# PeihaoChen/RSPNet

Hardware: AMD Instinct MI355X
Metric: clips/sec pretext step (c3d 16x112x112, B=32/GPU) (higher is better)
Workload: dtype f32

## Files before the change

rspnet_amd/csrc/common.h:

```cpp
#pragma once
#include <hip/hip_runtime.h>
#include <stdint.h>
#include <stdio.h>
#include <stdlib.h>
#include <string.h>
#include <tuple>

#include "rspnet_hip.h"

typedef float floatx16 __attribute__((ext_vector_type(16)));
typedef float floatx4 __attribute__((ext_vector_type(4)));

#define RSP_WAVE 64

void rsp_set_error(const char* msg);
void rsp_note_reset(void);
void rsp_note_kernel(const char* fmt, ...);

static inline int rsp_check_launch(const char* what) {
  hipError_t e = hipGetLastError();
  if (e != hipSuccess) {
    char buf[256];
    snprintf(buf, sizeof buf, "%.*s: %s", (int)strcspn(what, "<"), what, hipGetErrorString(e));
    rsp_set_error(buf);
    return RSP_ELAUNCH;
  }
  return RSP_OK;
}

#define RSP_CONV_OPTIONS(X)                                                             \
  X(OPT_NARROW_MAX_TILES, "narrow_max_tiles", "RSP_NARROW_MAX_TILES", 0, 512)           \
  X(OPT_NARROW32_MAX_UNITS, "narrow32_max_units", "RSP_NARROW32_MAX_UNITS", 0, 256)     \
  X(OPT_TALL_MIN_TILES, "tall_min_tiles", "RSP_TALL_MIN_TILES", 0, 0)                   \
  X(OPT_TWO_LEVEL_MIN_CHUNKS, "two_level_min_chunks", "RSP_TWO_LEVEL_MIN_CHUNKS", 0, 0) \
  X(OPT_DIRECT_MAX_TILES, "direct_max_tiles", "RSP_DIRECT_MAX_TILES", 0, 0)             \
  X(OPT_NO_PERSIST, "no_persist", "RSP_NO_PERSIST", 1, 0)                               \
  X(OPT_NO_HALF_BLOCK, "no_half_block", "RSP_NO_HALF_BLOCK", 1, 0)                      \
  X(OPT_NO_PAD_SKIP, "no_pad_skip", "RSP_NO_PAD_SKIP", 1, 0)                            \
  X(OPT_NO_DMAJOR, "no_dmajor", "RSP_NO_DMAJOR", 1, 0)                                  \
  X(OPT_NO_TM_SKIP, "no_tm_skip", "RSP_NO_TM_SKIP", 1, 0)                               \
  X(OPT_NO_MULTI_SPLIT, "no_multi_split", "RSP_NO_MULTI_SPLIT", 1, 0)
#define RSP_OPTION_ID(id, name, env, flag, dflt) id,
enum RspConvOption { RSP_CONV_OPTIONS(RSP_OPTION_ID) RSP_OPT_COUNT };
#undef RSP_OPTION_ID
int rsp_conv_option(RspConvOption id);

template <auto KERNEL, class... Args, class... Note>
int rsp_launch_lds(dim3 grid, size_t lds, size_t lds_max, hipStream_t s, const std::tuple<Args...>& args, const char* fmt, Note... note) {
  static bool attr_set = false;
  if (!attr_set) {
    (void)hipFuncSetAttribute(reinterpret_cast<const void*>(KERNEL), hipFuncAttributeMaxDynamicSharedMemorySize, (int)lds_max);
    attr_set = true;
  }
  rsp_note_kernel(fmt, note...);
  std::apply([&](const auto&... a) { hipLaunchKernelGGL(KERNEL, grid, dim3(256), lds, s, a...); }, args);
  return rsp_check_launch(fmt);
}

#define RSP_REQUIRE(cond, msg)     \
  do {                             \
    if (!(cond)) {                 \
      rsp_set_error(msg);          \
      return RSP_EINVAL;           \
    }                              \
  } while (0)

static inline size_t rsp_align_up(size_t v, size_t a) { return (v + a - 1) / a * a; }
static inline int rsp_cdiv(int64_t a, int64_t b) { return (int)((a + b - 1) / b); }
static inline bool rsp_aligned16(const void* p) { return (((uintptr_t)p) & 15) == 0; }

__device__ __forceinline__ int rsp_xcd_remap(int bid, int nwg) {
  const int q = nwg >> 3, r = nwg & 7;
  const int xcd = bid & 7;
  const int base = xcd < r ? xcd * (q + 1) : r * (q + 1) + (xcd - r) * q;
  return base + (bid >> 3);
}

__device__ __forceinline__ float rsp_wave_sum(float v) {
#pragma unroll
  for (int o = 32; o > 0; o >>= 1) v += __shfl_xor(v, o);
  return v;
}
__device__ __forceinline__ int rsp_wave_sum_i(int v) {
#pragma unroll
  for (int o = 32; o > 0; o >>= 1) v += __shfl_xor(v, o);
  return v;
}
__device__ __forceinline__ double rsp_wave_sum_d(double v) {
#pragma unroll
  for (int o = 32; o > 0; o >>= 1) v += __shfl_xor(v, o);
  return v;
}
__device__ __forceinline__ float rsp_wave_max(float v) {
#pragma unroll
  for (int o = 32; o > 0; o >>= 1) v = fmaxf(v, __shfl_xor(v, o));
  return v;
}

__device__ __forceinline__ float rsp_max_nan(float best, float v) { return __builtin_elementwise_maximum(best, v); }
__device__ __forceinline__ float rsp_relu(float z) { return __builtin_elementwise_maximum(z, 0.f); }
__device__ __forceinline__ bool rsp_relu_blocks(float z) { return z <= 0.f; }
__device__ __forceinline__ bool rsp_max_takes(float v, float best) { return v > best || v != v; }
__device__ __forceinline__ bool rsp_max_displaced(bool earlier, float v, float mine) {
  const bool vn = v != v, mn = mine != mine;
  return earlier ? (!mn && (vn || v >= mine)) : (vn || (!mn && v > mine));
}

struct FastDiv {
  unsigned mul;
  unsigned shr;
  int d;
};

static inline FastDiv fastdiv_make(int d) {
  FastDiv f = {0u, 0u, d};
  if (d <= 1) return f;
  int s = 0;
  while ((1ll << s) < d) ++s;
  const unsigned long long pw = 1ull << (31 + s);
  f.mul = (unsigned)((pw + (unsigned long long)d - 1) / (unsigned long long)d);
  f.shr = (unsigned)(s - 1);
  return f;
}

__device__ __forceinline__ int fastdiv(int n, const FastDiv f) {
  return f.mul ? (int)(__umulhi((unsigned)n, f.mul) >> f.shr) : n;
}
```

rspnet_amd/csrc/conv_stem.hip:

```cpp
#include "conv_stem.h"

#include <mutex>
#include <unordered_map>

namespace {

struct StemParams {
  const float* __restrict__ x;
  const float* __restrict__ w;
  const float* __restrict__ bias;
  float* __restrict__ y;
  float* __restrict__ stat;
  int N, Di, Hi, Wi, Do, Ho, Wo;
  int kT, kH, kW, sT, sH, sW, pT, pH, pW;
  int Cout, out_ld;
  int tw_shift;
  int HT, WT, WTh, WTL;
  int npix, npix_r;
  int FR;
  int ntaps, nchunks;
  int tiles_h, tiles_w, tiles;
  unsigned x_bytes, w_bytes;
  int wide;
  float* __restrict__ ymax;
  float* __restrict__ ymin;
  int pool_ld;
};

struct StemBias {
  floatx4 w[2];
  float n[2];
};

__device__ __forceinline__ StemBias stem_bias(const float* __restrict__ bias, int Cout, bool wide, int lane) {
  StemBias b;
#pragma unroll
  for (int j = 0; j < 2; ++j) {
    b.w[j] = floatx4{0.f, 0.f, 0.f, 0.f};
    b.n[j] = 0.f;
    const int cw = 32 * j + 4 * (lane & 7), cn = 32 * j + (lane & 31);
    if (bias && wide && cw < Cout) b.w[j] = *reinterpret_cast<const floatx4*>(bias + cw);
    if (bias && !wide && cn < Cout) b.n[j] = bias[cn];
  }
  asm volatile("" : "+v"(b.w[0]), "+v"(b.w[1]), "+v"(b.n[0]), "+v"(b.n[1]));
  return b;
}

__device__ __forceinline__ void stem_store_wide(const StemParams& p, const floatx16 (&acc)[2], float* stage ,
                                                const long long* rowaddr , int wave, int lane, const StemBias& b) {
  const int l32 = lane & 31, h = lane >> 5;
  const int q = lane & 7, rbase = lane >> 3;
#pragma unroll
  for (int j = 0; j < 2; ++j) {
    const int col = 32 * j + 4 * q;
#pragma unroll
    for (int r = 0; r < 2; ++r) {
#pragma unroll
      for (int e = 0; e < 8; ++e) stage[((e >> 2) * 8 + h * 4 + (e & 3)) * 32 + l32] = acc[j][8 * r + e];
#pragma unroll
      for (int i = 0; i < 2; ++i) {
        const int rl = rbase + 8 * i;
        const floatx4 v = *reinterpret_cast<const floatx4*>(stage + rl * 32 + 4 * q);
        const long long addr = rowaddr[wave * 32 + 16 * r + rl];
        if (addr >= 0 && col < p.Cout) *reinterpret_cast<floatx4*>(p.y + addr + col) = v + b.w[j];
      }
    }
  }
}

__device__ __forceinline__ void stem_store_pooled(const StemParams& p, const floatx16 (&acc)[2], float* stage ,
                                                  int n, int to, int h0, int w0, int wave, int lane, const StemBias& b) {
  const int l32 = lane & 31, h = lane >> 5;
  const int q = lane & 15, kr = lane >> 4;
  long long addr[2];
#pragma unroll
  for (int i = 0; i < 2; ++i) {
    const int ho = h0 + 2 * wave, wo = w0 + 2 * (kr + 4 * i);
    addr[i] = (ho < p.Ho && wo < p.Wo && 4 * q < p.Cout)
                  ? ((((long long)n * p.Do + to) * (p.Ho >> 1) + (ho >> 1)) * (p.Wo >> 1) + (wo >> 1)) * p.pool_ld + 4 * q
                  : -1;
  }
#pragma unroll
  for (int o = 0; o < 2; ++o) {
#pragma unroll
    for (int j = 0; j < 2; ++j)
#pragma unroll
      for (int e0 = 0; e0 < 8; e0 += 2) {
        const float v0 = acc[j][e0] + b.n[j], v1 = acc[j][e0 + 1] + b.n[j], v2 = acc[j][e0 + 8] + b.n[j], v3 = acc[j][e0 + 9] + b.n[j];
        const float r = o == 0 ? __builtin_elementwise_maximum(__builtin_elementwise_maximum(v0, v1), __builtin_elementwise_maximum(v2, v3))
                               : __builtin_elementwise_minimum(__builtin_elementwise_minimum(v0, v1), __builtin_elementwise_minimum(v2, v3));
        stage[((e0 >> 2) * 4 + h * 2 + ((e0 & 3) >> 1)) * 64 + 32 * j + l32] = r;
      }
    float* dst = o == 0 ? p.ymax : p.ymin;
#pragma unroll
    for (int i = 0; i < 2; ++i) {
      const floatx4 v = *reinterpret_cast<const floatx4*>(stage + (kr + 4 * i) * 64 + 4 * q);
      if (addr[i] >= 0) *reinterpret_cast<floatx4*>(dst + addr[i]) = v;
    }
  }
}

template <int G, int NS>
__global__ __launch_bounds__(256, 2) void stem_kernel(const StemParams p) {
  constexpr int TCH = 2 * G;
  constexpr int BU = TCH * 64;
  constexpr int BI = (BU + 255) / 256;
  typedef __attribute__((address_space(3))) void* lptr_t;
  extern __shared__ __attribute__((aligned(16))) unsigned char smem_raw[];
  float* halo = reinterpret_cast<float*>(smem_raw);
  float* Bs = halo + p.FR * p.npix_r * 4;
  int* taptab = reinterpret_cast<int*>(Bs + 2 * BU * 4);
  long long* rowaddr = reinterpret_cast<long long*>(taptab + p.nchunks * TCH);

  const int t = threadIdx.x;
  const int lane = t & 63;
  const int wave = __builtin_amdgcn_readfirstlane(t >> 6);
  const int l32 = lane & 31, h = lane >> 5;

  const int tile = rsp_xcd_remap(blockIdx.x, gridDim.x);
  const int wb = tile % p.tiles_w;
  int q0 = tile / p.tiles_w;
  const int hb = q0 % p.tiles_h;
  q0 /= p.tiles_h;
  const int to = q0 % p.Do;
  const int n = q0 / p.Do;
  const int TW = 1 << p.tw_shift, TH = 128 >> p.tw_shift;
  const int h0 = hb * TH, w0 = wb * TW;
  const StemBias bias = stem_bias(p.bias, p.Cout, p.wide != 0, lane);

  const int khw = p.kH * p.kW;
  for (int i = t; i < p.nchunks * TCH; i += 256) {
    int off = 0;
    if (i < p.ntaps) {
      const int kw = i % p.kW, r = i / p.kW;
      const int kh = r % p.kH, kt = r / p.kH;
      const int col = p.sW == 2 ? (kw & 1) * p.WTh + (kw >> 1) : kw;
      off = (((kt % p.FR) * p.npix_r) + kh * p.WTL + col) * 16;
    }
    taptab[i] = off;
  }

  unsigned hrel[4];
#pragma unroll
  for (int i = 0; i < 4; ++i) {
    const int q = i * 256 + t;
    unsigned r = 0xffffffffu;
    if (q < p.npix) {
      const int hyy = q / p.WTL, cc = q - hyy * p.WTL;
      const int wxp = p.sW == 2 ? (cc < p.WTh ? 2 * cc : 2 * (cc - p.WTh) + 1) : cc;
      const int hi = h0 * p.sH - p.pH + hyy, wi = w0 * p.sW - p.pW + wxp;
      if (wxp < p.WT && (unsigned)hi < (unsigned)p.Hi && (unsigned)wi < (unsigned)p.Wi) r = (unsigned)((hi * p.Wi + wi) * 16);
    }
    hrel[i] = r;
  }

  __amdgpu_buffer_rsrc_t rsrc_x = __builtin_amdgcn_make_buffer_rsrc(const_cast<float*>(p.x), 0, (int)p.x_bytes, 0x00020000);
  __amdgpu_buffer_rsrc_t rsrc_w = __builtin_amdgcn_make_buffer_rsrc(const_cast<float*>(p.w), 0, (int)p.w_bytes, 0x00020000);

  auto load_frame = [&](int f) {
    const int ti = to * p.sT - p.pT + f;
    const bool okf = (unsigned)ti < (unsigned)p.Di;
    const unsigned fbase = (unsigned)(((long long)(n * p.Di + (okf ? ti : 0)) * p.Hi * p.Wi) * 16);
    const int slot = f % p.FR;
#pragma unroll
    for (int i = 0; i < 4; ++i) {
      if (i * 256 + wave * 64 < p.npix_r) {
        const unsigned off = (okf & (hrel[i] != 0xffffffffu)) ? fbase + hrel[i] : 0xffffffffu;
        float* dst = halo + (slot * p.npix_r + i * 256 + wave * 64) * 4;
        __builtin_amdgcn_raw_ptr_buffer_load_lds(rsrc_x, (lptr_t)dst, 16, off, 0, 0, 0);
      }
    }
  };
  auto load_weights = [&](int c, int buf) {
#pragma unroll
    for (int i = 0; i < BI; ++i) {
      if (i * 256 + wave * 64 < BU) {
        const unsigned off = ((unsigned)c * BU + i * 256 + t) * 16u;
        float* dst = Bs + (buf * BU + i * 256 + wave * 64) * 4;
        __builtin_amdgcn_raw_ptr_buffer_load_lds(rsrc_w, (lptr_t)dst, 16, off, 0, 0, 0);
      }
    }
  };
  auto frame_hi = [&](int c) { return min(p.kT - 1, (c * TCH + TCH - 1) / khw); };

  int loaded = frame_hi(0);
  for (int f = 0; f <= loaded; ++f) load_frame(f);
  load_weights(0, 0);
  __syncthreads();

  const int m = wave * 32 + l32;
  const int hy = m >> p.tw_shift, wx = m & (TW - 1);
  const char* arow = reinterpret_cast<const char*>(halo) + ((hy * p.sH) * p.WTL + wx) * 16;
  int toff[G];
#pragma unroll
  for (int g = 0; g < G; ++g) toff[g] = taptab[2 * g + h];

  floatx16 acc[2];
#pragma unroll
  for (int j = 0; j < 2; ++j)
#pragma unroll
    for (int e = 0; e < 16; ++e) acc[j][e] = 0.f;

  int buf = 0;
  for (int c = 0; c < p.nchunks; ++c) {
    const bool more = c + 1 < p.nchunks;
    floatx4 af[G], bf[G][2];
#pragma unroll
    for (int g = 0; g < G; ++g) af[g] = *reinterpret_cast<const floatx4*>(arow + toff[g]);
    const float* bb = Bs + buf * BU * 4 + (h * 64 + l32) * 4;
#pragma unroll
    for (int g = 0; g < G; ++g)
#pragma unroll
      for (int j = 0; j < 2; ++j) bf[g][j] = *reinterpret_cast<const floatx4*>(bb + (2 * g * 64 + 32 * j) * 4);
    int toffn[G];
#pragma unroll
    for (int g = 0; g < G; ++g) toffn[g] = more ? taptab[(c + 1) * TCH + 2 * g + h] : 0;
    if (more) {
      load_weights(c + 1, buf ^ 1);
      const int fh = frame_hi(c + 1);
      while (loaded < fh) load_frame(++loaded);
    }
#pragma unroll
    for (int g = 0; g < G; ++g)
#pragma unroll
      for (int s = 0; s < NS; ++s)
#pragma unroll
        for (int j = 0; j < 2; ++j) acc[j] = __builtin_amdgcn_mfma_f32_32x32x2f32(af[g][s], bf[g][j][s], acc[j], 0, 0, 0);
    __builtin_amdgcn_sched_barrier(0);
    __syncthreads();
    buf ^= 1;
#pragma unroll
    for (int g = 0; g < G; ++g) toff[g] = toffn[g];
  }

  if (t < 128) {
    const int ry = t >> p.tw_shift, rx = t & (TW - 1);
    const int ho = h0 + ry, wo = w0 + rx;
    rowaddr[t] = (ho < p.Ho && wo < p.Wo) ? ((((long long)n * p.Do + to) * p.Ho + ho) * p.Wo + wo) * p.out_ld : -1;
  }
  __syncthreads();
  float* red = Bs;
  if (p.wide) stem_store_wide(p, acc, Bs + 512 + wave * 512, rowaddr, wave, lane, bias);
#pragma unroll
  for (int j = 0; j < 2; ++j) {
    const int col = 32 * j + l32;
    const float bv = bias.n[j];
    float s = 0.f, ss = 0.f;
#pragma unroll
    for (int e = 0; e < 16; ++e) {
      const long long addr = rowaddr[wave * 32 + (e >> 2) * 8 + h * 4 + (e & 3)];
      const float v = addr >= 0 ? acc[j][e] : 0.f;
      if (!p.wide && addr >= 0 && col < p.Cout) p.y[addr + col] = v + bv;
      s += v;
      ss = fmaf(v, v, ss);
    }
    s += __shfl_xor(s, 32);
    ss += __shfl_xor(ss, 32);
    if (h == 0) {
      red[(wave * 64 + col) * 2 + 0] = s;
      red[(wave * 64 + col) * 2 + 1] = ss;
    }
  }
  if (p.stat) {
    __syncthreads();
    if (t < 64 && t < p.Cout) {
      float s = 0.f, ss = 0.f;
#pragma unroll
      for (int w = 0; w < 4; ++w) {
        s += red[(w * 64 + t) * 2 + 0];
        ss += red[(w * 64 + t) * 2 + 1];
      }
      float* o = p.stat + ((long long)tile * p.Cout + t) * 2;
      o[0] = s;
      o[1] = ss;
    }
  }
}

template <int G, bool WIDE, int NS, bool POOL = false>
__global__ __launch_bounds__(256, 2) void stem_resident_kernel(const StemParams p) {
  constexpr int TCH = 2 * G;
  constexpr int BU = TCH * 64;
  constexpr int BI = (BU + 255) / 256;
  typedef __attribute__((address_space(3))) void* lptr_t;
  extern __shared__ __attribute__((aligned(16))) unsigned char smem_raw[];
  const int hsz = p.FR * p.npix_r * 4;
  float* halo = reinterpret_cast<float*>(smem_raw);
  float* Bs = halo + 2 * hsz;
  int* taptab = reinterpret_cast<int*>(Bs + p.nchunks * BU * 4);
  long long* rowaddr = reinterpret_cast<long long*>(taptab + p.nchunks * TCH);
  float* red = reinterpret_cast<float*>(rowaddr + 128);

  const int t = threadIdx.x;
  const int lane = t & 63;
  const int wave = __builtin_amdgcn_readfirstlane(t >> 6);
  const int l32 = lane & 31, h = lane >> 5;
  const int TW = 1 << p.tw_shift, TH = 128 >> p.tw_shift;

  for (int i = t; i < p.nchunks * TCH; i += 256) {
    int off = 0;
    if (i < p.ntaps) {
      const int kw = i % p.kW, r = i / p.kW;
      const int kh = r % p.kH, kt = r / p.kH;
      const int col = p.sW == 2 ? (kw & 1) * p.WTh + (kw >> 1) : kw;
      off = ((kt * p.npix_r) + kh * p.WTL + col) * 16;
    }
    taptab[i] = off;
  }
  __amdgpu_buffer_rsrc_t rsrc_x = __builtin_amdgcn_make_buffer_rsrc(const_cast<float*>(p.x), 0, (int)p.x_bytes, 0x00020000);
  __amdgpu_buffer_rsrc_t rsrc_w = __builtin_amdgcn_make_buffer_rsrc(const_cast<float*>(p.w), 0, (int)p.w_bytes, 0x00020000);
  for (int c = 0; c < p.nchunks; ++c) {
#pragma unroll
    for (int i = 0; i < BI; ++i) {
      if (i * 256 + wave * 64 < BU) {
        const unsigned off = ((unsigned)c * BU + i * 256 + t) * 16u;
        float* dst = Bs + (c * BU + i * 256 + wave * 64) * 4;
        __builtin_amdgcn_raw_ptr_buffer_load_lds(rsrc_w, (lptr_t)dst, 16, off, 0, 0, 0);
      }
    }
  }
  int hyy[4], wxp[4];
#pragma unroll
  for (int i = 0; i < 4; ++i) {
    const int q = i * 256 + t;
    hyy[i] = -(1 << 20);
    wxp[i] = 0;
    if (q < p.npix) {
      const int r = q / p.WTL, cc = q - r * p.WTL;
      const int wx_ = p.sW == 2 ? (cc < p.WTh ? 2 * cc : 2 * (cc - p.WTh) + 1) : cc;
      if (wx_ < p.WT) {
        hyy[i] = r;
        wxp[i] = wx_;
      }
    }
  }
  auto issue_halo = [&](int tile, int buf) {
    const int wb = tile % p.tiles_w;
    int q0 = tile / p.tiles_w;
    const int hb = q0 % p.tiles_h;
    q0 /= p.tiles_h;
    const int to = q0 % p.Do, n = q0 / p.Do;
    const int hi0 = hb * TH * p.sH - p.pH, wi0 = wb * TW * p.sW - p.pW;
    unsigned hrel[4];
#pragma unroll
    for (int i = 0; i < 4; ++i) {
      const int hi = hi0 + hyy[i], wi = wi0 + wxp[i];
      hrel[i] = ((unsigned)hi < (unsigned)p.Hi && (unsigned)wi < (unsigned)p.Wi) ? (unsigned)((hi * p.Wi + wi) * 16) : 0xffffffffu;
    }
    for (int f = 0; f < p.kT; ++f) {
      const int ti = to * p.sT - p.pT + f;
      const bool okf = (unsigned)ti < (unsigned)p.Di;
      const unsigned fbase = (unsigned)(((long long)(n * p.Di + (okf ? ti : 0)) * p.Hi * p.Wi) * 16);
#pragma unroll
      for (int i = 0; i < 4; ++i) {
        if (i * 256 + wave * 64 < p.npix_r) {
          const unsigned off = (okf & (hrel[i] != 0xffffffffu)) ? fbase + hrel[i] : 0xffffffffu;
          float* dst = halo + buf * hsz + (f * p.npix_r + i * 256 + wave * 64) * 4;
          __builtin_amdgcn_raw_ptr_buffer_load_lds(rsrc_x, (lptr_t)dst, 16, off, 0, 0, 0);
        }
      }
    }
  };

  const int m = wave * 32 + l32;
  const int rowoff = (((m >> p.tw_shift) * p.sH) * p.WTL + (m & (TW - 1))) * 16;
  const StemBias bias = stem_bias(p.bias, p.Cout, WIDE, lane);

  int cur = 0;
  if ((int)blockIdx.x < p.tiles) issue_halo(blockIdx.x, 0);
  for (int tile = blockIdx.x; tile < p.tiles; tile += gridDim.x) {
    __syncthreads();
    const int next = tile + gridDim.x;
    const char* arow = reinterpret_cast<const char*>(halo + cur * hsz) + rowoff;
    floatx16 acc[2];
#pragma unroll
    for (int j = 0; j < 2; ++j)
#pragma unroll
      for (int e = 0; e < 16; ++e) acc[j][e] = 0.f;
    for (int c = 0; c < p.nchunks; ++c) {
      floatx4 af[G], bf[G][2];
#pragma unroll
      for (int g = 0; g < G; ++g) af[g] = *reinterpret_cast<const floatx4*>(arow + taptab[c * TCH + 2 * g + h]);
      const float* bb = Bs + c * BU * 4 + (h * 64 + l32) * 4;
#pragma unroll
      for (int g = 0; g < G; ++g)
#pragma unroll
        for (int j = 0; j < 2; ++j) bf[g][j] = *reinterpret_cast<const floatx4*>(bb + (2 * g * 64 + 32 * j) * 4);
      if (c == p.nchunks - 1 && next < p.tiles) issue_halo(next, cur ^ 1);
#pragma unroll
      for (int g = 0; g < G; ++g)
#pragma unroll
        for (int s = 0; s < NS; ++s)
#pragma unroll
          for (int j = 0; j < 2; ++j) acc[j] = __builtin_amdgcn_mfma_f32_32x32x2f32(af[g][s], bf[g][j][s], acc[j], 0, 0, 0);
    }
    const int wb = tile % p.tiles_w;
    int q0 = tile / p.tiles_w;
    const int hb = q0 % p.tiles_h;
    q0 /= p.tiles_h;
    const int to = q0 % p.Do, n = q0 / p.Do;
    if (t < 128) {
      const int ho = hb * TH + (t >> p.tw_shift), wo = wb * TW + (t & (TW - 1));
      rowaddr[t] = (ho < p.Ho && wo < p.Wo) ? ((((long long)n * p.Do + to) * p.Ho + ho) * p.Wo + wo) * p.out_ld : -1;
    }
    __syncthreads();
    if (WIDE) stem_store_wide(p, acc, halo + cur * hsz + wave * 512, rowaddr, wave, lane, bias);
    if (POOL) stem_store_pooled(p, acc, halo + cur * hsz + wave * 512, n, to, hb * TH, wb * TW, wave, lane, bias);
#pragma unroll
    for (int j = 0; j < 2; ++j) {
      const int col = 32 * j + l32;
      const float bv = bias.n[j];
      float s = 0.f, ss = 0.f;
#pragma unroll
      for (int e = 0; e < 16; ++e) {
        const long long addr = rowaddr[wave * 32 + (e >> 2) * 8 + h * 4 + (e & 3)];
        const float v = addr >= 0 ? acc[j][e] : 0.f;
        if (!WIDE && !POOL && addr >= 0 && col < p.Cout) p.y[addr + col] = v + bv;
        s += v;
        ss = fmaf(v, v, ss);
      }
      s += __shfl_xor(s, 32);
      ss += __shfl_xor(ss, 32);
      if (h == 0) {
        red[(wave * 64 + col) * 2 + 0] = s;
        red[(wave * 64 + col) * 2 + 1] = ss;
      }
    }
    if (p.stat) {
      __syncthreads();
      if (t < 64 && t < p.Cout) {
        float s = 0.f, ss = 0.f;
#pragma unroll
        for (int w = 0; w < 4; ++w) {
          s += red[(w * 64 + t) * 2 + 0];
          ss += red[(w * 64 + t) * 2 + 1];
        }
        float* o = p.stat + ((long long)tile * p.Cout + t) * 2;
        o[0] = s;
        o[1] = ss;
      }
    }
    cur ^= 1;
  }
}

__global__ void stem_pack_kernel(const float* __restrict__ w, float* __restrict__ out, int Cout, int kT, int kH, int kW,
                                 int ntaps, long long total) {
  for (long long i = blockIdx.x * (long long)blockDim.x + threadIdx.x; i < total; i += (long long)gridDim.x * blockDim.x) {
    const int ci = (int)(i & 3), n = (int)((i >> 2) & 63), tap = (int)(i >> 8);
    float v = 0.f;
    if (tap < ntaps && n < Cout) {
      const int kw = tap % kW, r = tap / kW;
      const int kh = r % kH, kt = r / kH;
      v = w[((((long long)n * 4 + ci) * kT + kt) * kH + kh) * kW + kw];
    }
    out[i] = v;
  }
}

struct StemPlan {
  bool ok;
  int G, TCH, nchunks, tw_shift, HT, WT, WTh, WTL, npix, npix_r, FR, tiles_h, tiles_w;
  bool resident;
  bool wide_ok;
  long long tiles;
  size_t lds;
};

StemPlan stem_plan(const rsp_conv3d_desc* d) {
  StemPlan s;
  memset(&s, 0, sizeof s);
  if (d->Cin != 4 || d->in_ld != 4 || d->Cout > 64 || d->out_ld < d->Cout) return s;
  if (d->sW < 1 || d->sW > 2 || d->sH < 1 || d->sH > 2) return s;
  const int ntaps = d->kT * d->kH * d->kW;
  if (ntaps > 343) return s;
  if ((unsigned long long)d->N * d->Di * d->Hi * d->Wi * 16ull >= 0xF0000000ull) return s;
  const long long waste16 = (long long)rsp_cdiv(d->Ho, 8) * 8 * rsp_cdiv(d->Wo, 16) * 16;
  const long long waste8 = (long long)rsp_cdiv(d->Ho, 16) * 16 * rsp_cdiv(d->Wo, 8) * 8;
  s.tw_shift = waste8 < waste16 ? 3 : 4;
  const long long covered = waste8 < waste16 ? waste8 : waste16;
  if (ntaps > 64 && covered * 100 > (long long)d->Ho * d->Wo * 104) return s;
  const int TW = 1 << s.tw_shift, TH = 128 >> s.tw_shift;
  s.HT = (TH - 1) * d->sH + d->kH;
  s.WT = (TW - 1) * d->sW + d->kW;
  s.WTh = (s.WT + 1) / 2;
  s.WTL = d->sW == 2 ? 2 * s.WTh : s.WT;
  s.npix = s.HT * s.WTL;
  if (s.npix > 1024) return s;
  s.npix_r = (s.npix + 63) / 64 * 64;
  s.FR = d->kT < 3 ? d->kT : 3;
  int best = 0, best_pad = 1 << 30;
  const int cand[3] = {8, 7, 5};
  for (int i = 0; i < 3; ++i) {
    const int tch = 2 * cand[i];
    if (d->kT > 3 && d->kH * d->kW < 2 * tch) continue;
    const int pad = rsp_cdiv(ntaps, tch) * tch;
    if (pad < best_pad) {
      best_pad = pad;
      best = cand[i];
    }
  }
  if (!best) return s;
  s.G = best;
  s.TCH = 2 * best;
  s.nchunks = rsp_cdiv(ntaps, s.TCH);
  s.tiles_h = rsp_cdiv(d->Ho, TH);
  s.tiles_w = rsp_cdiv(d->Wo, TW);
  s.tiles = (long long)d->N * d->Do * s.tiles_h * s.tiles_w;
  if (s.tiles >= (1ll << 31)) return s;
  const size_t lds_res = (size_t)2 * d->kT * s.npix_r * 16 + (size_t)s.nchunks * s.TCH * 1024 + (size_t)s.nchunks * s.TCH * 4 +
                         128 * 8 + 2048;
  s.resident = d->kT <= 3 && lds_res <= 78 * 1024;
  s.lds = s.resident ? lds_res
                     : (size_t)s.FR * s.npix_r * 16 + (size_t)2 * s.TCH * 1024 + (size_t)s.nchunks * s.TCH * 4 + 128 * 8;
  if (s.lds > 150 * 1024) return s;
  s.wide_ok = d->Cout % 4 == 0 && d->out_ld % 4 == 0 && (!s.resident || ((size_t)d->kT * s.npix_r * 16 >= 8192 && s.G != 8));
  s.ok = true;
  return s;
}

std::mutex g_three_mu;
std::unordered_map<const void*, bool> g_three;

bool stem_three_channels(const void* w_packed) {
  std::lock_guard<std::mutex> lk(g_three_mu);
  auto it = g_three.find(w_packed);
  return it != g_three.end() && it->second;
}

template <int G, int NS>
int launch_stem(const StemParams& p, const StemPlan& pl, hipStream_t s) {
  static bool attr_set = false;
  if (!attr_set) {
    (void)hipFuncSetAttribute(reinterpret_cast<const void*>(&stem_kernel<G, NS>), hipFuncAttributeMaxDynamicSharedMemorySize,
                              150 * 1024);
    attr_set = true;
  }
  if (pl.resident) {
    static bool attr_set_r = false;
    if (!attr_set_r) {
      (void)hipFuncSetAttribute(reinterpret_cast<const void*>(&stem_resident_kernel<G, true, NS>),
                                hipFuncAttributeMaxDynamicSharedMemorySize, 80 * 1024);
      (void)hipFuncSetAttribute(reinterpret_cast<const void*>(&stem_resident_kernel<G, false, NS>),
                                hipFuncAttributeMaxDynamicSharedMemorySize, 80 * 1024);
      attr_set_r = true;
    }
    long long per_cu = (160 * 1024) / (long long)pl.lds;
    per_cu = per_cu > 3 ? 3 : per_cu;
    const long long grid = pl.tiles < 256 * per_cu ? pl.tiles : 256 * per_cu;
    rsp_note_kernel(p.wide ? "stem_resident_kernel<%d, true, %d>" : "stem_resident_kernel<%d, false, %d>", G, NS);
    if (p.wide) hipLaunchKernelGGL((stem_resident_kernel<G, true, NS>), dim3((unsigned)grid), dim3(256), pl.lds, s, p);
    else hipLaunchKernelGGL((stem_resident_kernel<G, false, NS>), dim3((unsigned)grid), dim3(256), pl.lds, s, p);
    return rsp_check_launch("stem_resident_kernel");
  }
  rsp_note_kernel("stem_kernel<%d, %d>", G, NS);
  hipLaunchKernelGGL((stem_kernel<G, NS>), dim3((unsigned)pl.tiles), dim3(256), pl.lds, s, p);
  return rsp_check_launch("stem_kernel");
}

}

bool rsp_stem_applicable(const rsp_conv3d_desc* d) { return stem_plan(d).ok; }

int rsp_stem_tiles(const rsp_conv3d_desc* d) { return (int)stem_plan(d).tiles; }

const char* rsp_stem_kernel_name(const rsp_conv3d_desc* d) {
  const StemPlan pl = stem_plan(d);
  if (pl.resident && pl.wide_ok)
    return pl.G == 8 ? "stem_resident_kernel<8, true, 3>" : (pl.G == 7 ? "stem_resident_kernel<7, true, 3>" : "stem_resident_kernel<5, true, 3>");
  if (pl.resident)
    return pl.G == 8 ? "stem_resident_kernel<8, false, 3>" : (pl.G == 7 ? "stem_resident_kernel<7, false, 3>" : "stem_resident_kernel<5, false, 3>");
  return pl.G == 8 ? "stem_kernel<8, 3>" : (pl.G == 7 ? "stem_kernel<7, 3>" : "stem_kernel<5, 3>");
}

void rsp_stem_note_packed(const void* w_packed, bool three_channels) {
  std::lock_guard<std::mutex> lk(g_three_mu);
  if (three_channels) g_three[w_packed] = true;
  else g_three.erase(w_packed);
}

void rsp_stem_forget_packed(const void* w_packed) {
  std::lock_guard<std::mutex> lk(g_three_mu);
  g_three.erase(w_packed);
}

size_t rsp_stem_packed_elems(const rsp_conv3d_desc* d) {
  const StemPlan pl = stem_plan(d);
  return (size_t)pl.nchunks * pl.TCH * 256;
}

int rsp_stem_pack(const rsp_conv3d_desc* d, const float* w_ref, float* w_packed, hipStream_t s) {
  const StemPlan pl = stem_plan(d);
  const long long total = (long long)pl.nchunks * pl.TCH * 256;
  const int blocks = (int)((total + 255) / 256 > 2048 ? 2048 : (total + 255) / 256);
  rsp_stem_note_packed(w_packed, false);
  hipLaunchKernelGGL(stem_pack_kernel, dim3(blocks), dim3(256), 0, s, w_ref, w_packed, d->Cout, d->kT, d->kH, d->kW,
                     d->kT * d->kH * d->kW, total);
  return rsp_check_launch("stem_pack_kernel");
}

static StemParams stem_params(const rsp_conv3d_desc* d, const StemPlan& pl, const float* x, const float* w_packed, const float* bias,
                              float* stat_partials) {
  StemParams p;
  memset(&p, 0, sizeof p);
  p.x = x; p.w = w_packed; p.bias = bias; p.stat = stat_partials;
  p.N = d->N; p.Di = d->Di; p.Hi = d->Hi; p.Wi = d->Wi; p.Do = d->Do; p.Ho = d->Ho; p.Wo = d->Wo;
  p.kT = d->kT; p.kH = d->kH; p.kW = d->kW; p.sT = d->sT; p.sH = d->sH; p.sW = d->sW;
  p.pT = d->pT; p.pH = d->pH; p.pW = d->pW;
  p.Cout = d->Cout; p.out_ld = d->out_ld;
  p.tw_shift = pl.tw_shift;
  p.HT = pl.HT; p.WT = pl.WT; p.WTh = pl.WTh; p.WTL = pl.WTL;
  p.npix = pl.npix; p.npix_r = pl.npix_r; p.FR = pl.FR;
  p.ntaps = d->kT * d->kH * d->kW; p.nchunks = pl.nchunks;
  p.tiles_h = pl.tiles_h; p.tiles_w = pl.tiles_w; p.tiles = (int)pl.tiles;
  p.x_bytes = (unsigned)((unsigned long long)d->N * d->Di * d->Hi * d->Wi * 16ull);
  p.w_bytes = (unsigned)((size_t)pl.nchunks * pl.TCH * 1024);
  return p;
}

int rsp_stem_fwd(const rsp_conv3d_desc* d, const float* x, const float* w_packed, const float* bias, float* y,
                 float* stat_partials, hipStream_t s) {
  const StemPlan pl = stem_plan(d);
  RSP_REQUIRE(pl.ok, "rsp_stem_fwd: descriptor not on the stem path");
  RSP_REQUIRE(rsp_aligned16(x) && rsp_aligned16(w_packed), "rsp_conv3d_fwd: 4-channel input and packed weight must be 16-byte aligned");
  StemParams p = stem_params(d, pl, x, w_packed, bias, stat_partials);
  p.y = y;
  p.wide = pl.wide_ok && rsp_aligned16(y) && (!bias || rsp_aligned16(bias));
  if (stem_three_channels(w_packed)) {
    switch (pl.G) {
      case 8: return launch_stem<8, 3>(p, pl, s);
      case 7: return launch_stem<7, 3>(p, pl, s);
      default: return launch_stem<5, 3>(p, pl, s);
    }
  }
  switch (pl.G) {
    case 8: return launch_stem<8, 4>(p, pl, s);
    case 7: return launch_stem<7, 4>(p, pl, s);
    default: return launch_stem<5, 4>(p, pl, s);
  }
}

static bool stem_pooled_ok(const rsp_conv3d_desc* d, const StemPlan& pl) {
  return pl.ok && pl.resident && pl.wide_ok && pl.tw_shift == 4 && d->Ho % 2 == 0 && d->Wo % 2 == 0 && d->Cout % 4 == 0;
}

template <int G, int NS>
static int launch_stem_pooled(const StemParams& p, const StemPlan& pl, hipStream_t s) {
  long long per_cu = (160 * 1024) / (long long)pl.lds;
  per_cu = per_cu > 3 ? 3 : per_cu;
  const long long grid = pl.tiles < 256 * per_cu ? pl.tiles : 256 * per_cu;
  return rsp_launch_lds<stem_resident_kernel<G, false, NS, true>>(dim3((unsigned)grid), pl.lds, 80 * 1024, s, std::tie(p),
                                                                  "stem_resident_kernel<%d, false, %d, true>", G, NS);
}

bool rsp_stem_pooled_applicable(const rsp_conv3d_desc* d) { return stem_pooled_ok(d, stem_plan(d)); }

int rsp_stem_pooled_fwd(const rsp_conv3d_desc* d, const float* x, const float* w_packed, const float* bias, float* y_max, float* y_min,
                        float* stat_partials, hipStream_t stream) {
  const StemPlan pl = stem_plan(d);
  RSP_REQUIRE(stem_pooled_ok(d, pl), "rsp_conv3d_stem_pooled_fwd: descriptor not covered (rsp_conv3d_stem_pooled_applicable)");
  RSP_REQUIRE(rsp_aligned16(x) && rsp_aligned16(w_packed) && rsp_aligned16(y_max) && rsp_aligned16(y_min),
              "rsp_conv3d_stem_pooled_fwd: input, packed weight and both outputs must be 16-byte aligned");
  StemParams p = stem_params(d, pl, x, w_packed, bias, stat_partials);
  p.ymax = y_max; p.ymin = y_min; p.pool_ld = d->Cout;
  if (stem_three_channels(w_packed)) {
    switch (pl.G) {
      case 7: return launch_stem_pooled<7, 3>(p, pl, stream);
      default: return launch_stem_pooled<5, 3>(p, pl, stream);
    }
  }
  switch (pl.G) {
    case 7: return launch_stem_pooled<7, 4>(p, pl, stream);
    default: return launch_stem_pooled<5, 4>(p, pl, stream);
  }
}
```

Measured before the change: 355.6.

## Add full-patch stem path with buffer stores and fewer barriers

Adds a FULL template variant of the resident stem conv kernel for shapes whose output tiles always lie fully in bounds with Cout=64. That variant drops the per-tile rowaddr table and writes through buffer-resource stores addressed from a per-tile base offset. Tile coordinates are now advanced incrementally instead of recomputed with divisions. The stat partial reduction is double-buffered and deferred by one tile so a full __syncthreads per tile can become a partial vmcnt wait plus s_barrier. This costs extra LDS for the second reduction buffer and adds template variants, and it relies on 32-bit byte offsets into the output.

```diff
diff --git a/rspnet_amd/csrc/common.h b/rspnet_amd/csrc/common.h
--- a/rspnet_amd/csrc/common.h
+++ b/rspnet_amd/csrc/common.h
@@ -39,7 +39,8 @@
   X(OPT_NO_PAD_SKIP, "no_pad_skip", "RSP_NO_PAD_SKIP", 1, 0)                            \
   X(OPT_NO_DMAJOR, "no_dmajor", "RSP_NO_DMAJOR", 1, 0)                                  \
   X(OPT_NO_TM_SKIP, "no_tm_skip", "RSP_NO_TM_SKIP", 1, 0)                               \
-  X(OPT_NO_MULTI_SPLIT, "no_multi_split", "RSP_NO_MULTI_SPLIT", 1, 0)
+  X(OPT_NO_MULTI_SPLIT, "no_multi_split", "RSP_NO_MULTI_SPLIT", 1, 0)                   \
+  X(OPT_NO_STEM_FULL_PATCH, "no_stem_full_patch", "RSP_NO_STEM_FULL_PATCH", 1, 0)
 #define RSP_OPTION_ID(id, name, env, flag, dflt) id,
 enum RspConvOption { RSP_CONV_OPTIONS(RSP_OPTION_ID) RSP_OPT_COUNT };
 #undef RSP_OPTION_ID
diff --git a/rspnet_amd/csrc/conv_stem.hip b/rspnet_amd/csrc/conv_stem.hip
--- a/rspnet_amd/csrc/conv_stem.hip
+++ b/rspnet_amd/csrc/conv_stem.hip
@@ -25,7 +25,45 @@
   float* __restrict__ ymax;
   float* __restrict__ ymin;
   int pool_ld;
+  unsigned out_bytes;
 };
+
+struct StemOut {
+  __amdgpu_buffer_rsrc_t rs, rs2;
+  unsigned voff;
+  unsigned base;
+};
+typedef unsigned uintx4 __attribute__((ext_vector_type(4)));
+
+struct StemPatch {
+  int n, to, hb, wb;
+};
+
+__device__ __forceinline__ StemPatch stem_patch_of(int tile, const StemParams& p) {
+  StemPatch c;
+  c.wb = tile % p.tiles_w;
+  int q0 = tile / p.tiles_w;
+  c.hb = q0 % p.tiles_h;
+  q0 /= p.tiles_h;
+  c.to = q0 % p.Do;
+  c.n = q0 / p.Do;
+  return c;
+}
+
+__device__ __forceinline__ StemPatch stem_patch_next(StemPatch c, const StemPatch& step, const StemParams& p) {
+  c.wb += step.wb;
+  if (c.wb >= p.tiles_w) { c.wb -= p.tiles_w; ++c.hb; }
+  c.hb += step.hb;
+  if (c.hb >= p.tiles_h) { c.hb -= p.tiles_h; ++c.to; }
+  c.to += step.to;
+  if (c.to >= p.Do) { c.to -= p.Do; ++c.n; }
+  c.n += step.n;
+  return c;
+}
+
+__device__ __forceinline__ void stem_store16(const floatx4 v, __amdgpu_buffer_rsrc_t rs, unsigned voff, unsigned soff) {
+  __builtin_amdgcn_raw_buffer_store_b128(__builtin_bit_cast(uintx4, v), rs, (int)(voff + soff), 0, 0);
+}
 
 struct StemBias {
   floatx4 w[2];
@@ -46,8 +84,10 @@
   return b;
 }
 
+template <bool FULL>
 __device__ __forceinline__ void stem_store_wide(const StemParams& p, const floatx16 (&acc)[2], float* stage ,
-                                                const long long* rowaddr , int wave, int lane, const StemBias& b) {
+                                                const long long* rowaddr , int wave, int lane, const StemBias& b,
+                                                const StemOut& o) {
   const int l32 = lane & 31, h = lane >> 5;
   const int q = lane & 7, rbase = lane >> 3;
 #pragma unroll
@@ -61,6 +101,12 @@
       for (int i = 0; i < 2; ++i) {
         const int rl = rbase + 8 * i;
         const floatx4 v = *reinterpret_cast<const floatx4*>(stage + rl * 32 + 4 * q);
+        if (FULL) {
+          const int Ru = wave * 32 + 16 * r + 8 * i;
+          const unsigned u = (unsigned)(((Ru >> p.tw_shift) * p.Wo + (Ru & ((1 << p.tw_shift) - 1))) * p.out_ld) * 4u;
+          stem_store16(v + b.w[j], o.rs, o.voff + 128u * j, o.base + u);
+          continue;
+        }
         const long long addr = rowaddr[wave * 32 + 16 * r + rl];
         if (addr >= 0 && col < p.Cout) *reinterpret_cast<floatx4*>(p.y + addr + col) = v + b.w[j];
       }
@@ -68,13 +114,16 @@
   }
 }
 
+template <bool FULL>
 __device__ __forceinline__ void stem_store_pooled(const StemParams& p, const floatx16 (&acc)[2], float* stage ,
-                                                  int n, int to, int h0, int w0, int wave, int lane, const StemBias& b) {
+                                                  int n, int to, int h0, int w0, int wave, int lane, const StemBias& b,
+                                                  const StemOut& out) {
   const int l32 = lane & 31, h = lane >> 5;
   const int q = lane & 15, kr = lane >> 4;
   long long addr[2];
 #pragma unroll
   for (int i = 0; i < 2; ++i) {
+    if (FULL) continue;
     const int ho = h0 + 2 * wave, wo = w0 + 2 * (kr + 4 * i);
     addr[i] = (ho < p.Ho && wo < p.Wo && 4 * q < p.Cout)
                   ? ((((long long)n * p.Do + to) * (p.Ho >> 1) + (ho >> 1)) * (p.Wo >> 1) + (wo >> 1)) * p.pool_ld + 4 * q
@@ -95,6 +144,10 @@
 #pragma unroll
     for (int i = 0; i < 2; ++i) {
       const floatx4 v = *reinterpret_cast<const floatx4*>(stage + (kr + 4 * i) * 64 + 4 * q);
+      if (FULL) {
+        stem_store16(v, o == 0 ? out.rs : out.rs2, out.voff, out.base + (unsigned)((wave * (p.Wo >> 1) + 4 * i) * p.pool_ld) * 4u);
+        continue;
+      }
       if (addr[i] >= 0) *reinterpret_cast<floatx4*>(dst + addr[i]) = v;
     }
   }
@@ -240,7 +293,7 @@
   }
   __syncthreads();
   float* red = Bs;
-  if (p.wide) stem_store_wide(p, acc, Bs + 512 + wave * 512, rowaddr, wave, lane, bias);
+  if (p.wide) stem_store_wide<false>(p, acc, Bs + 512 + wave * 512, rowaddr, wave, lane, bias, StemOut());
 #pragma unroll
   for (int j = 0; j < 2; ++j) {
     const int col = 32 * j + l32;
@@ -277,7 +330,7 @@
   }
 }
 
-template <int G, bool WIDE, int NS, bool POOL = false>
+template <int G, bool WIDE, int NS, bool POOL = false, bool FULL = false>
 __global__ __launch_bounds__(256, 2) void stem_resident_kernel(const StemParams p) {
   constexpr int TCH = 2 * G;
   constexpr int BU = TCH * 64;
@@ -334,13 +387,9 @@
       }
     }
   }
-  auto issue_halo = [&](int tile, int buf) {
-    const int wb = tile % p.tiles_w;
-    int q0 = tile / p.tiles_w;
-    const int hb = q0 % p.tiles_h;
-    q0 /= p.tiles_h;
-    const int to = q0 % p.Do, n = q0 / p.Do;
-    const int hi0 = hb * TH * p.sH - p.pH, wi0 = wb * TW * p.sW - p.pW;
+  auto issue_halo = [&](const StemPatch& pt, int buf) {
+    const int to = pt.to, n = pt.n;
+    const int hi0 = pt.hb * TH * p.sH - p.pH, wi0 = pt.wb * TW * p.sW - p.pW;
     unsigned hrel[4];
 #pragma unroll
     for (int i = 0; i < 4; ++i) {
@@ -366,11 +415,40 @@
   const int rowoff = (((m >> p.tw_shift) * p.sH) * p.WTL + (m & (TW - 1))) * 16;
   const StemBias bias = stem_bias(p.bias, p.Cout, WIDE, lane);
 
-  int cur = 0;
-  if ((int)blockIdx.x < p.tiles) issue_halo(blockIdx.x, 0);
-  for (int tile = blockIdx.x; tile < p.tiles; tile += gridDim.x) {
-    __syncthreads();
+  StemOut out;
+  out.voff = out.base = 0;
+  if (FULL) {
+    out.rs = __builtin_amdgcn_make_buffer_rsrc(POOL ? p.ymax : p.y, 0, (int)p.out_bytes, 0x00020000);
+    out.rs2 = __builtin_amdgcn_make_buffer_rsrc(POOL ? p.ymin : p.y, 0, (int)p.out_bytes, 0x00020000);
+    out.voff = POOL   ? (unsigned)((lane >> 4) * p.pool_ld + 4 * (lane & 15)) * 4u
+               : WIDE ? (unsigned)((lane >> 3) * p.out_ld + 4 * (lane & 7)) * 4u
+                      : (unsigned)(4 * h * p.out_ld + l32) * 4u;
+  }
+  auto write_stat = [&](int tile_, const float* r) {
+    if (t < 64 && t < p.Cout) {
+      float s = 0.f, ss = 0.f;
+#pragma unroll
+      for (int w = 0; w < 4; ++w) {
+        s += r[(w * 64 + t) * 2 + 0];
+        ss += r[(w * 64 + t) * 2 + 1];
+      }
+      float* o = p.stat + ((long long)tile_ * p.Cout + t) * 2;
+      o[0] = s;
+      o[1] = ss;
+    }
+  };
+  constexpr int NST = POOL ? 4 : (WIDE ? 8 : 32);
+
+  int cur = 0, pb = 0;
+  int tile = blockIdx.x, done = -1;
+  const StemPatch step = stem_patch_of(gridDim.x, p);
+  StemPatch pt = stem_patch_of(tile, p);
+  if (tile < p.tiles) issue_halo(pt, 0);
+  __syncthreads();
+  while (tile < p.tiles) {
+    if (p.stat && done >= 0) write_stat(done, red + (pb ^ 1) * 512);
     const int next = tile + gridDim.x;
+    const StemPatch ptn = stem_patch_next(pt, step, p);
     const char* arow = reinterpret_cast<const char*>(halo + cur * hsz) + rowoff;
     floatx16 acc[2];
 #pragma unroll
@@ -386,7 +464,7 @@
       for (int g = 0; g < G; ++g)
 #pragma unroll
         for (int j = 0; j < 2; ++j) bf[g][j] = *reinterpret_cast<const floatx4*>(bb + (2 * g * 64 + 32 * j) * 4);
-      if (c == p.nchunks - 1 && next < p.tiles) issue_halo(next, cur ^ 1);
+      if (c == p.nchunks - 1 && next < p.tiles) issue_halo(ptn, cur ^ 1);
 #pragma unroll
       for (int g = 0; g < G; ++g)
 #pragma unroll
@@ -394,18 +472,27 @@
 #pragma unroll
           for (int j = 0; j < 2; ++j) acc[j] = __builtin_amdgcn_mfma_f32_32x32x2f32(af[g][s], bf[g][j][s], acc[j], 0, 0, 0);
     }
-    const int wb = tile % p.tiles_w;
-    int q0 = tile / p.tiles_w;
-    const int hb = q0 % p.tiles_h;
-    q0 /= p.tiles_h;
-    const int to = q0 % p.Do, n = q0 / p.Do;
-    if (t < 128) {
-      const int ho = hb * TH + (t >> p.tw_shift), wo = wb * TW + (t & (TW - 1));
-      rowaddr[t] = (ho < p.Ho && wo < p.Wo) ? ((((long long)n * p.Do + to) * p.Ho + ho) * p.Wo + wo) * p.out_ld : -1;
-    }
-    __syncthreads();
-    if (WIDE) stem_store_wide(p, acc, halo + cur * hsz + wave * 512, rowaddr, wave, lane, bias);
-    if (POOL) stem_store_pooled(p, acc, halo + cur * hsz + wave * 512, n, to, hb * TH, wb * TW, wave, lane, bias);
+    const int n = pt.n, to = pt.to, hb = pt.hb, wb = pt.wb;
+    if (!FULL) {
+      if (lane < 32) {
+        const int r = wave * 32 + lane;
+        const int ho = hb * TH + (r >> p.tw_shift), wo = wb * TW + (r & (TW - 1));
+        rowaddr[r] = (ho < p.Ho && wo < p.Wo) ? ((((long long)n * p.Do + to) * p.Ho + ho) * p.Wo + wo) * p.out_ld : -1;
+      }
+      __builtin_amdgcn_wave_barrier();
+    } else if (POOL) {
+      out.base = (unsigned)(((((n * p.Do + to) * (p.Ho >> 1) + hb * 4) * (p.Wo >> 1)) + wb * 8) * p.pool_ld) * 4u;
+    } else {
+      out.base = (unsigned)(((((n * p.Do + to) * p.Ho + hb * TH) * p.Wo) + wb * TW) * p.out_ld) * 4u;
+    }
+    if (WIDE || POOL) {
+      asm volatile("s_waitcnt lgkmcnt(0)" ::: "memory");
+      __builtin_amdgcn_s_barrier();
+      asm volatile("" ::: "memory");
+    }
+    if (WIDE) stem_store_wide<FULL>(p, acc, halo + cur * hsz + wave * 512, rowaddr, wave, lane, bias, out);
+    if (POOL) stem_store_pooled<FULL>(p, acc, halo + cur * hsz + wave * 512, n, to, hb * TH, wb * TW, wave, lane, bias, out);
+    float* redw = red + pb * 512;
 #pragma unroll
     for (int j = 0; j < 2; ++j) {
       const int col = 32 * j + l32;
@@ -413,34 +500,46 @@
       float s = 0.f, ss = 0.f;
 #pragma unroll
       for (int e = 0; e < 16; ++e) {
-        const long long addr = rowaddr[wave * 32 + (e >> 2) * 8 + h * 4 + (e & 3)];
-        const float v = addr >= 0 ? acc[j][e] : 0.f;
-        if (!WIDE && !POOL && addr >= 0 && col < p.Cout) p.y[addr + col] = v + bv;
+        float v;
+        if (FULL) {
+          v = acc[j][e];
+          if (!WIDE && !POOL) {
+            const int Ru = wave * 32 + (e >> 2) * 8 + (e & 3);
+            const unsigned u = (unsigned)(((Ru >> p.tw_shift) * p.Wo + (Ru & (TW - 1))) * p.out_ld) * 4u;
+            __builtin_amdgcn_raw_buffer_store_b32(__float_as_uint(v + bv), out.rs, (int)(out.voff + 128u * j), (int)(out.base + u), 0);
+          }
+        } else {
+          const long long addr = rowaddr[wave * 32 + (e >> 2) * 8 + h * 4 + (e & 3)];
+          v = addr >= 0 ? acc[j][e] : 0.f;
+          if (!WIDE && !POOL && addr >= 0 && col < p.Cout) p.y[addr + col] = v + bv;
+        }
         s += v;
         ss = fmaf(v, v, ss);
       }
       s += __shfl_xor(s, 32);
       ss += __shfl_xor(ss, 32);
       if (h == 0) {
-        red[(wave * 64 + col) * 2 + 0] = s;
-        red[(wave * 64 + col) * 2 + 1] = ss;
-      }
-    }
-    if (p.stat) {
+        redw[(wave * 64 + col) * 2 + 0] = s;
+        redw[(wave * 64 + col) * 2 + 1] = ss;
+      }
+    }
+    done = tile;
+    tile = next;
+    pt = ptn;
+    cur ^= 1;
+    pb ^= 1;
+    if (tile >= p.tiles) break;
+    if (FULL) {
+      asm volatile("s_waitcnt vmcnt(%0) lgkmcnt(0)" ::"n"(NST) : "memory");
+      __builtin_amdgcn_s_barrier();
+      asm volatile("" ::: "memory");
+    } else {
       __syncthreads();
-      if (t < 64 && t < p.Cout) {
-        float s = 0.f, ss = 0.f;
-#pragma unroll
-        for (int w = 0; w < 4; ++w) {
-          s += red[(w * 64 + t) * 2 + 0];
-          ss += red[(w * 64 + t) * 2 + 1];
-        }
-        float* o = p.stat + ((long long)tile * p.Cout + t) * 2;
-        o[0] = s;
-        o[1] = ss;
-      }
-    }
-    cur ^= 1;
+    }
+  }
+  if (p.stat) {
+    __syncthreads();
+    if (done >= 0) write_stat(done, red + (pb ^ 1) * 512);
   }
 }
 
@@ -509,7 +608,7 @@
   s.tiles = (long long)d->N * d->Do * s.tiles_h * s.tiles_w;
   if (s.tiles >= (1ll << 31)) return s;
   const size_t lds_res = (size_t)2 * d->kT * s.npix_r * 16 + (size_t)s.nchunks * s.TCH * 1024 + (size_t)s.nchunks * s.TCH * 4 +
-                         128 * 8 + 2048;
+                         128 * 8 + 2 * 2048;
   s.resident = d->kT <= 3 && lds_res <= 78 * 1024;
   s.lds = s.resident ? lds_res
                      : (size_t)s.FR * s.npix_r * 16 + (size_t)2 * s.TCH * 1024 + (size_t)s.nchunks * s.TCH * 4 + 128 * 8;
@@ -528,30 +627,36 @@
   return it != g_three.end() && it->second;
 }
 
+bool stem_full_patch(const rsp_conv3d_desc* d, const StemPlan& pl, unsigned long long bytes) {
+  const int TW = 1 << pl.tw_shift, TH = 128 >> pl.tw_shift;
+  return pl.resident && d->Ho % TH == 0 && d->Wo % TW == 0 && d->Cout == 64 && bytes < (1ull << 32) &&
+         !rsp_conv_option(OPT_NO_STEM_FULL_PATCH);
+}
+
+long long stem_resident_grid(const StemPlan& pl) {
+  long long per_cu = (160 * 1024) / (long long)pl.lds;
+  per_cu = per_cu > 3 ? 3 : per_cu;
+  return pl.tiles < 256 * per_cu ? pl.tiles : 256 * per_cu;
+}
+
+template <int G, bool WIDE, int NS, bool FULL>
+int launch_stem_resident(const StemParams& p, const StemPlan& pl, hipStream_t s) {
+  return rsp_launch_lds<stem_resident_kernel<G, WIDE, NS, false, FULL>>(
+      dim3((unsigned)stem_resident_grid(pl)), pl.lds, 80 * 1024, s, std::tie(p),
+      WIDE ? "stem_resident_kernel<%d, true, %d>" : "stem_resident_kernel<%d, false, %d>", G, NS);
+}
+
 template <int G, int NS>
-int launch_stem(const StemParams& p, const StemPlan& pl, hipStream_t s) {
+int launch_stem(const StemParams& p, const StemPlan& pl, bool full, hipStream_t s) {
+  if (pl.resident) {
+    if (p.wide) return full ? launch_stem_resident<G, true, NS, true>(p, pl, s) : launch_stem_resident<G, true, NS, false>(p, pl, s);
+    return full ? launch_stem_resident<G, false, NS, true>(p, pl, s) : launch_stem_resident<G, false, NS, false>(p, pl, s);
+  }
   static bool attr_set = false;
   if (!attr_set) {
     (void)hipFuncSetAttribute(reinterpret_cast<const void*>(&stem_kernel<G, NS>), hipFuncAttributeMaxDynamicSharedMemorySize,
                               150 * 1024);
     attr_set = true;
-  }
-  if (pl.resident) {
-    static bool attr_set_r = false;
-    if (!attr_set_r) {
-      (void)hipFuncSetAttribute(reinterpret_cast<const void*>(&stem_resident_kernel<G, true, NS>),
-                                hipFuncAttributeMaxDynamicSharedMemorySize, 80 * 1024);
-      (void)hipFuncSetAttribute(reinterpret_cast<const void*>(&stem_resident_kernel<G, false, NS>),
-                                hipFuncAttributeMaxDynamicSharedMemorySize, 80 * 1024);
-      attr_set_r = true;
-    }
-    long long per_cu = (160 * 1024) / (long long)pl.lds;
-    per_cu = per_cu > 3 ? 3 : per_cu;
-    const long long grid = pl.tiles < 256 * per_cu ? pl.tiles : 256 * per_cu;
-    rsp_note_kernel(p.wide ? "stem_resident_kernel<%d, true, %d>" : "stem_resident_kernel<%d, false, %d>", G, NS);
-    if (p.wide) hipLaunchKernelGGL((stem_resident_kernel<G, true, NS>), dim3((unsigned)grid), dim3(256), pl.lds, s, p);
-    else hipLaunchKernelGGL((stem_resident_kernel<G, false, NS>), dim3((unsigned)grid), dim3(256), pl.lds, s, p);
-    return rsp_check_launch("stem_resident_kernel");
   }
   rsp_note_kernel("stem_kernel<%d, %d>", G, NS);
   hipLaunchKernelGGL((stem_kernel<G, NS>), dim3((unsigned)pl.tiles), dim3(256), pl.lds, s, p);
@@ -626,17 +731,20 @@
   StemParams p = stem_params(d, pl, x, w_packed, bias, stat_partials);
   p.y = y;
   p.wide = pl.wide_ok && rsp_aligned16(y) && (!bias || rsp_aligned16(bias));
+  const unsigned long long y_bytes = (((unsigned long long)d->N * d->Do * d->Ho * d->Wo - 1) * d->out_ld + d->Cout) * 4ull;
+  const bool full = stem_full_patch(d, pl, y_bytes);
+  p.out_bytes = full ? (unsigned)y_bytes : 0u;
   if (stem_three_channels(w_packed)) {
     switch (pl.G) {
-      case 8: return launch_stem<8, 3>(p, pl, s);
-      case 7: return launch_stem<7, 3>(p, pl, s);
-      default: return launch_stem<5, 3>(p, pl, s);
+      case 8: return launch_stem<8, 3>(p, pl, full, s);
+      case 7: return launch_stem<7, 3>(p, pl, full, s);
+      default: return launch_stem<5, 3>(p, pl, full, s);
     }
   }
   switch (pl.G) {
-    case 8: return launch_stem<8, 4>(p, pl, s);
-    case 7: return launch_stem<7, 4>(p, pl, s);
-    default: return launch_stem<5, 4>(p, pl, s);
+    case 8: return launch_stem<8, 4>(p, pl, full, s);
+    case 7: return launch_stem<7, 4>(p, pl, full, s);
+    default: return launch_stem<5, 4>(p, pl, full, s);
   }
 }
 
@@ -645,12 +753,13 @@
 }
 
 template <int G, int NS>
-static int launch_stem_pooled(const StemParams& p, const StemPlan& pl, hipStream_t s) {
-  long long per_cu = (160 * 1024) / (long long)pl.lds;
-  per_cu = per_cu > 3 ? 3 : per_cu;
-  const long long grid = pl.tiles < 256 * per_cu ? pl.tiles : 256 * per_cu;
-  return rsp_launch_lds<stem_resident_kernel<G, false, NS, true>>(dim3((unsigned)grid), pl.lds, 80 * 1024, s, std::tie(p),
-                                                                  "stem_resident_kernel<%d, false, %d, true>", G, NS);
+static int launch_stem_pooled(const StemParams& p, const StemPlan& pl, bool full, hipStream_t s) {
+  const dim3 grid((unsigned)stem_resident_grid(pl));
+  if (full)
+    return rsp_launch_lds<stem_resident_kernel<G, false, NS, true, true>>(grid, pl.lds, 80 * 1024, s, std::tie(p),
+                                                                          "stem_resident_kernel<%d, false, %d, true>", G, NS);
+  return rsp_launch_lds<stem_resident_kernel<G, false, NS, true, false>>(grid, pl.lds, 80 * 1024, s, std::tie(p),
+                                                                         "stem_resident_kernel<%d, false, %d, true>", G, NS);
 }
 
 bool rsp_stem_pooled_applicable(const rsp_conv3d_desc* d) { return stem_pooled_ok(d, stem_plan(d)); }
@@ -663,14 +772,17 @@
               "rsp_conv3d_stem_pooled_fwd: input, packed weight and both outputs must be 16-byte aligned");
   StemParams p = stem_params(d, pl, x, w_packed, bias, stat_partials);
   p.ymax = y_max; p.ymin = y_min; p.pool_ld = d->Cout;
+  const unsigned long long pool_bytes = (unsigned long long)d->N * d->Do * (d->Ho / 2) * (d->Wo / 2) * d->Cout * 4ull;
+  const bool full = stem_full_patch(d, pl, pool_bytes);
+  p.out_bytes = full ? (unsigned)pool_bytes : 0u;
   if (stem_three_channels(w_packed)) {
     switch (pl.G) {
-      case 7: return launch_stem_pooled<7, 3>(p, pl, stream);
-      default: return launch_stem_pooled<5, 3>(p, pl, stream);
+      case 7: return launch_stem_pooled<7, 3>(p, pl, full, stream);
+      default: return launch_stem_pooled<5, 3>(p, pl, full, stream);
     }
   }
   switch (pl.G) {
-    case 7: return launch_stem_pooled<7, 4>(p, pl, stream);
-    default: return launch_stem_pooled<5, 4>(p, pl, stream);
-  }
-}
+    case 7: return launch_stem_pooled<7, 4>(p, pl, full, stream);
+    default: return launch_stem_pooled<5, 4>(p, pl, full, stream);
+  }
+}
```

After: 356.1 (median of 6 runs). Within noise of the previous version (+0.1%).
